# atomicarchitects/equiformer

Measured on AMD Instinct MI355X. Metric: molecules/sec (train step) QM9 L_max=2, 6 blocks, higher is better.
Workload: dtype f32; 1 GPU; QM9 graph_attention_transformer_nonlinear_l2 train step (radius graph + fwd + L1 + bwd + AdamW), 128 molecules/GPU x 18 atoms, r=5.0, num_basis=128, alpha_drop=0.2; global_batch=128, nodes_per_gpu=2304, edges_per_gpu=25354, parallelism=dp1, matrix_mode=split, hip_graph=True, hip_graph_replays=463, hip_graph_eager_steps=3

## Files before the change

equiformer_amd/csrc/gemmx.hip:

```cpp
#include <climits>
#include "sfcx_common.h"

namespace {

constexpr int GX_BK = 32;
constexpr int GX_LDK = 40;
constexpr int GX_T = 64;
constexpr int GX_ROW = GX_T * GX_LDK;
constexpr int GX_MAXP = 24;

typedef __bf16 bf16x4_t __attribute__((ext_vector_type(4)));

struct GRows {
  const float* base;
  int d, ld, inner;
};

struct GXP {
  GRows A, B, C;
  const float* bias;
  float* cs;
  float* Cw;
  int ldc;
  int M, N, K;
  int accumulate, kind;
  int vecA, vecB;
  int steps_per_split;
};
static_assert(sizeof(GXP) * GX_MAXP + 4 * (2 * GX_MAXP + 3) <= 4000, "kernarg segment");
struct GXGroup {
  int n;
  int woff[GX_MAXP + 1];
  GXP p[GX_MAXP];
};

__device__ __forceinline__ int flat_problem(const GXGroup& g, int b) {
  int pi = 0;
#pragma unroll
  for (int j = 1; j < GX_MAXP; ++j) pi += (int)((unsigned)(g.woff[j] - 1 - b) >> 31);
  return pi;
}

template <int NP>
__device__ __forceinline__ void split_n(const float* v, int n, __bf16 (*p)[8]) {
#pragma unroll
  for (int j = 0; j < 8; ++j) {
    if (j >= n) break;
    float r = v[j];
#pragma unroll
    for (int q = 0; q < NP; ++q) {
      const __bf16 h = (__bf16)r;
      p[q][j] = h;
      if (q + 1 < NP) r = r - (float)h;
    }
  }
}

template <int NP>
struct LoaderKC {
  float4 v[2];
  long roff[2];
  bool rv[2];
  __device__ __forceinline__ void init(const GRows& R, int x0, int X) {
    const int xr0 = threadIdx.x >> 3;
#pragma unroll
    for (int pass = 0; pass < 2; ++pass) {
      const int x = x0 + xr0 + 32 * pass;
      rv[pass] = x < X;
      roff[pass] = row_off2(rv[pass] ? x : x0, R.d, R.ld, R.inner);
    }
  }
  int krem;
  template <bool VEC>
  __device__ __forceinline__ void issue(const GRows& R, int k0, int K) {
    const int k = k0 + 4 * (threadIdx.x & 7);
    krem = K - k;
    if constexpr (VEC) {
      const int kc = krem > 0 ? k : 0;
#pragma unroll
      for (int pass = 0; pass < 2; ++pass) v[pass] = *reinterpret_cast<const float4*>(R.base + roff[pass] + kc);
    } else {
#pragma unroll
      for (int pass = 0; pass < 2; ++pass) {
        const float* const p = R.base + roff[pass];
        v[pass] = make_float4(p[min(k, K - 1)], p[min(k + 1, K - 1)], p[min(k + 2, K - 1)], p[min(k + 3, K - 1)]);
      }
    }
  }
  __device__ __forceinline__ void commit(__bf16* __restrict__ T) const {
    const int kq = threadIdx.x & 7, xr0 = threadIdx.x >> 3;
#pragma unroll
    for (int pass = 0; pass < 2; ++pass) {
      float f[4] = {v[pass].x, v[pass].y, v[pass].z, v[pass].w};
#pragma unroll
      for (int e = 0; e < 4; ++e)
        if (!(rv[pass] && e < krem)) f[e] = 0.f;
      __bf16 p[NP][8];
      split_n<NP>(f, 4, p);
#pragma unroll
      for (int q = 0; q < NP; ++q)
        *reinterpret_cast<bf16x4_t*>(T + q * GX_ROW + (xr0 + 32 * pass) * GX_LDK + 4 * kq) =
            bf16x4_t{p[q][0], p[q][1], p[q][2], p[q][3]};
    }
  }
};

template <int NP>
struct LoaderKS {
  float v[8];
  float cs, cc;
  int kleft;
  int kb, q, rem;
  __device__ __forceinline__ void init(const GRows& R, int k_first) {
    cs = 0.f, cc = 0.f;
    kb = k_first + 8 * (threadIdx.x >> 6);
    q = kb / R.d;
    rem = kb - q * R.d;
  }
  __device__ __forceinline__ void issue(const GRows& R, int K, int x0, int X) {
    const int x = x0 + (threadIdx.x & 63);
    const bool xv = x < X;
    const int nv = K - kb;
    kleft = xv ? nv : -1;
    const float* const p = R.base + (xv ? x : x0) + (nv > 0 ? (long)q * R.ld + (long)rem * R.inner : 0L);
    const int wrap = R.ld - R.d * R.inner;
    int rel = 0, r = rem;
#pragma unroll
    for (int j = 0; j < 8; ++j) {
      v[j] = p[j < nv ? rel : 0];
      rel += R.inner;
      if (++r == R.d) r = 0, rel += wrap;
    }
    const int q32 = GX_BK / R.d, r32 = GX_BK - q32 * R.d;
    kb += GX_BK, q += q32, rem += r32;
    if (rem >= R.d) rem -= R.d, ++q;
  }
  __device__ __forceinline__ void commit(__bf16* __restrict__ T, bool want_cs) {
    const int x = threadIdx.x & 63, kg = threadIdx.x >> 6;
#pragma unroll
    for (int j = 0; j < 8; ++j)
      if (j >= kleft) v[j] = 0.f;
    if (want_cs) {
#pragma unroll
      for (int j = 0; j < 8; ++j) {
        const float y = v[j] - cc, t = cs + y;
        cc = (t - cs) - y, cs = t;
      }
    }
    __bf16 p[NP][8];
    split_n<NP>(v, 8, p);
#pragma unroll
    for (int q_ = 0; q_ < NP; ++q_)
      *reinterpret_cast<bf16x8*>(T + q_ * GX_ROW + x * GX_LDK + 8 * kg) =
          bf16x8{p[q_][0], p[q_][1], p[q_][2], p[q_][3], p[q_][4], p[q_][5], p[q_][6], p[q_][7]};
  }
};

template <int NA, int NB>
__device__ __forceinline__ void gx_mma(const __bf16* __restrict__ As, const __bf16* __restrict__ Bs, int wm0, int wn0,
                                       f32x16& acc) {
  const int lane = threadIdx.x & 63, r = lane & 31, hi = lane >> 5;
#pragma unroll
  for (int kt = 0; kt < GX_BK / 16; ++kt) {
    bf16x8 a[NA], b[NB];
#pragma unroll
    for (int q = 0; q < NA; ++q) a[q] = *reinterpret_cast<const bf16x8*>(As + q * GX_ROW + (wm0 + r) * GX_LDK + 16 * kt + 8 * hi);
#pragma unroll
    for (int q = 0; q < NB; ++q) b[q] = *reinterpret_cast<const bf16x8*>(Bs + q * GX_ROW + (wn0 + r) * GX_LDK + 16 * kt + 8 * hi);
    mma_terms<NA, NB>(a, b, acc);
  }
}

constexpr int GX_ST_LD = 36;
constexpr int GX_ST_FLOATS = 16 * GX_ST_LD;
template <typename RowPtr>
__device__ __forceinline__ void gx_store_tile16(const f32x16& acc, float* __restrict__ T, const int row0, const int M, const int col0,
                                                const int N, const bool accumulate, const int lane, RowPtr rowptr) {
  const int r = lane & 31, hi = lane >> 5, c4 = 4 * (lane & 7), rr = lane >> 3;
#pragma unroll
  for (int half = 0; half < 2; ++half) {
    __builtin_amdgcn_fence(__ATOMIC_ACQ_REL, "wavefront");
    __builtin_amdgcn_wave_barrier();
#pragma unroll
    for (int q8 = 0; q8 < 8; ++q8) T[((q8 & 3) + 8 * (q8 >> 2) + 4 * hi) * GX_ST_LD + r] = acc[8 * half + q8];
    __builtin_amdgcn_fence(__ATOMIC_ACQ_REL, "wavefront");
    __builtin_amdgcn_wave_barrier();
#pragma unroll
    for (int k = 0; k < 2; ++k) {
      const int lr = rr + 8 * k, grow = row0 + 16 * half + lr;
      f32x4 v = *reinterpret_cast<const f32x4*>(T + lr * GX_ST_LD + c4);
      if (grow < M && col0 + c4 < N) {
        float* const p = rowptr(grow) + (col0 + c4);
        if (accumulate) {
          const f32x4 o = *reinterpret_cast<const f32x4*>(p);
          v[0] += o[0], v[1] += o[1], v[2] += o[2], v[3] += o[3];
        }
        *reinterpret_cast<f32x4*>(p) = v;
      }
    }
  }
}

template <int MODE, int BKIND, bool VEC>
__global__ __launch_bounds__(256) void gemmx_rows_kernel(const GXGroup g_byval) {
  KERNARG_IN_PLACE(GXGroup);
  constexpr int NA = Planes<MODE>::A, NB = Planes<MODE>::W;
  const int pi = flat_problem(g, (int)blockIdx.x);
  const GXP& P = g.p[pi];
  const int local = (int)blockIdx.x - g.woff[pi], tiles_n = (P.N + GX_T - 1) / GX_T;
  const int mt = local / tiles_n;
  const int m0 = mt * GX_T, n0 = (local - mt * tiles_n) * GX_T;
  __shared__ __attribute__((aligned(16))) __bf16 As[2][NA * GX_ROW];
  __shared__ __attribute__((aligned(16))) __bf16 Bs[2][NB * GX_ROW];
  const int wave = threadIdx.x >> 6;
  const int wm0 = (wave >> 1) * 32, wn0 = (wave & 1) * 32;
  f32x16 acc;
#pragma unroll
  for (int q = 0; q < 16; ++q) acc[q] = 0.f;

  LoaderKC<NA> la;
  LoaderKC<NB> lbk;
  LoaderKS<NB> lbs;
  la.init(P.A, m0, P.M);
  la.template issue<VEC>(P.A, 0, P.K);
  if constexpr (BKIND == 1) {
    lbk.init(P.B, n0, P.N);
    lbk.template issue<VEC>(P.B, 0, P.K);
  } else {
    lbs.init(P.B, 0);
    lbs.issue(P.B, P.K, n0, P.N);
  }
  la.commit(As[0]);
  if constexpr (BKIND == 1) lbk.commit(Bs[0]);
  else lbs.commit(Bs[0], false);
  __syncthreads();
  int cur = 0;
  for (int k0 = 0; k0 < P.K; k0 += GX_BK) {
    const bool more = k0 + GX_BK < P.K;
    if (more) {
      la.template issue<VEC>(P.A, k0 + GX_BK, P.K);
      if constexpr (BKIND == 1) lbk.template issue<VEC>(P.B, k0 + GX_BK, P.K);
      else lbs.issue(P.B, P.K, n0, P.N);
    }
    gx_mma<NA, NB>(As[cur], Bs[cur], wm0, wn0, acc);
    if (more) {
      la.commit(As[cur ^ 1]);
      if constexpr (BKIND == 1) lbk.commit(Bs[cur ^ 1]);
      else lbs.commit(Bs[cur ^ 1], false);
    }
    __syncthreads();
    cur ^= 1;
  }

  const int lane = threadIdx.x & 63, r = lane & 31, hi = lane >> 5;
  const int col = n0 + wn0 + r;
  const float bv = (P.bias && col < P.N) ? P.bias[col] : 0.f;
  const bool flat_c = P.C.d == 1;
  const SmallDiv cdiv(P.C.d);
  float* const cbase = const_cast<float*>(P.C.base);
  const int rb = m0 + wm0 + 4 * hi;
  static_assert(sizeof(As) >= 4 * GX_ST_FLOATS * sizeof(float), "the operand stages double as the store tiles");
  if (((P.C.ld | P.C.inner | P.N) & 3) == 0 && (reinterpret_cast<size_t>(cbase) & 15) == 0) {
#pragma unroll
    for (int q = 0; q < 16; ++q) acc[q] += bv;
    gx_store_tile16(acc, reinterpret_cast<float*>(&As[0][0]) + wave * GX_ST_FLOATS, m0 + wm0, P.M, n0 + wn0, P.N, P.accumulate != 0,
                    lane, [&](const int grow) {
                      if (flat_c) return cbase + (long)grow * P.C.ld;
                      const int qd = grow / P.C.d;
                      return cbase + (long)qd * P.C.ld + (long)(grow - qd * P.C.d) * P.C.inner;
                    });
    return;
  }
  if (col >= P.N) return;
  long off0;
  int rem0 = 0;
  if (flat_c) {
    off0 = (long)rb * P.C.ld;
  } else {
    const int qb = rb / P.C.d;
    rem0 = rb - qb * P.C.d;
    off0 = (long)qb * P.C.ld;
  }
#pragma unroll
  for (int q = 0; q < 16; ++q) {
    const int dr = (q & 3) + 8 * (q >> 2);
    if (rb + dr < P.M) {
      long off;
      if (flat_c) {
        off = off0 + (long)dr * P.C.ld;
      } else {
        const int t = rem0 + dr, dq = cdiv.div(t);
        off = off0 + (long)dq * P.C.ld + (long)(t - dq * P.C.d) * P.C.inner;
      }
      float* p = cbase + off + col;
      float v = acc[q] + bv;
      if (P.accumulate) v += *p;
      *p = v;
    }
  }
}

constexpr int GW_K = 64;
constexpr int GW_LDK = GW_K + 8;
constexpr int GW_ROW = GX_T * GW_LDK;

template <int NP>
struct LoaderWide {
  float4 v[GW_K / 16];
  int kv;
  __device__ __forceinline__ void issue(const GRows& R, int x0, int X, int K, bool two_level) {
    const int row = x0 + (threadIdx.x >> 2), q = threadIdx.x & 3;
    const bool rv = row < X;
    kv = rv ? K : 0;
    const long off = two_level ? row_off2(rv ? row : x0, R.d, R.ld, R.inner) : (long)(rv ? row : x0) * R.ld;
#pragma unroll
    for (int j = 0; j < GW_K / 16; ++j) {
      const int k = 4 * (q + 4 * j);
      v[j] = *reinterpret_cast<const float4*>(R.base + off + (k < K ? k : 0));
    }
  }
  __device__ __forceinline__ void commit(__bf16* __restrict__ T) const {
    const int row = threadIdx.x >> 2, q = threadIdx.x & 3;
#pragma unroll
    for (int j = 0; j < GW_K / 16; ++j) {
      const bool ok = 4 * (q + 4 * j) < kv;
      const float f[4] = {ok ? v[j].x : 0.f, ok ? v[j].y : 0.f, ok ? v[j].z : 0.f, ok ? v[j].w : 0.f};
      __bf16 p[NP][8];
      split_n<NP>(f, 4, p);
#pragma unroll
      for (int pl = 0; pl < NP; ++pl)
        *reinterpret_cast<bf16x4_t*>(T + pl * GW_ROW + row * GW_LDK + 4 * (q + 4 * j)) = bf16x4_t{p[pl][0], p[pl][1], p[pl][2], p[pl][3]};
    }
  }
};

template <int MODE>
__global__ __launch_bounds__(256) void gemmx_rows_wide_kernel(const GXGroup g_byval) {
  KERNARG_IN_PLACE(GXGroup);
  constexpr int NA = Planes<MODE>::A, NB = Planes<MODE>::W;
  const GXP& P = g.p[blockIdx.z];
  const int m0 = blockIdx.x * GX_T;
  if (m0 >= P.M) return;
  __shared__ __attribute__((aligned(16))) __bf16 As[NA * GW_ROW];
  __shared__ __attribute__((aligned(16))) __bf16 Bs[NB * GW_ROW];
  __shared__ __attribute__((aligned(16))) float St[4 * GX_ST_FLOATS];
  const int wave = threadIdx.x >> 6, lane = threadIdx.x & 63, r = lane & 31, hi = lane >> 5;
  const int wm0 = (wave >> 1) * 32, wn0 = (wave & 1) * 32;
  LoaderWide<NA> la;
  LoaderWide<NB> lb;
  la.issue(P.A, m0, P.M, P.K, true);
  lb.issue(P.B, 0, P.N, P.K, false);
  la.commit(As);
  const bool flat_c = P.C.d == 1;
  const SmallDiv cdiv(P.C.d);
  float* const cbase = const_cast<float*>(P.C.base);
  const int rb = m0 + wm0 + 4 * hi;
  long off0;
  int rem0 = 0;
  if (flat_c) {
    off0 = (long)rb * P.C.ld;
  } else {
    const int qb = rb / P.C.d;
    rem0 = rb - qb * P.C.d;
    off0 = (long)qb * P.C.ld;
  }
  const int nkt = (P.K + 15) / 16;
  const bool vec_c = ((P.C.ld | P.C.inner | P.N) & 3) == 0 && (reinterpret_cast<size_t>(cbase) & 15) == 0;
  for (int n0 = 0; n0 < P.N; n0 += GX_T) {
    __syncthreads();
    lb.commit(Bs);
    __syncthreads();
    if (n0 + GX_T < P.N) lb.issue(P.B, n0 + GX_T, P.N, P.K, false);
    f32x16 acc;
#pragma unroll
    for (int q = 0; q < 16; ++q) acc[q] = 0.f;
#pragma unroll
    for (int kt = 0; kt < GW_K / 16; ++kt) {
      if (kt < nkt) {
        bf16x8 a[NA], b[NB];
#pragma unroll
        for (int q = 0; q < NA; ++q) a[q] = *reinterpret_cast<const bf16x8*>(As + q * GW_ROW + (wm0 + r) * GW_LDK + 16 * kt + 8 * hi);
#pragma unroll
        for (int q = 0; q < NB; ++q) b[q] = *reinterpret_cast<const bf16x8*>(Bs + q * GW_ROW + (wn0 + r) * GW_LDK + 16 * kt + 8 * hi);
        mma_terms<NA, NB>(a, b, acc);
      }
    }
    const int col = n0 + wn0 + r;
    if (vec_c) {
      const float bv = (P.bias && col < P.N) ? P.bias[col] : 0.f;
#pragma unroll
      for (int q = 0; q < 16; ++q) acc[q] += bv;
      gx_store_tile16(acc, St + wave * GX_ST_FLOATS, m0 + wm0, P.M, n0 + wn0, P.N, P.accumulate != 0, lane, [&](const int grow) {
        if (flat_c) return cbase + (long)grow * P.C.ld;
        const int qd = grow / P.C.d;
        return cbase + (long)qd * P.C.ld + (long)(grow - qd * P.C.d) * P.C.inner;
      });
    } else if (col < P.N) {
      const float bv = P.bias ? P.bias[col] : 0.f;
#pragma unroll
      for (int q = 0; q < 16; ++q) {
        const int dr = (q & 3) + 8 * (q >> 2);
        if (rb + dr < P.M) {
          long off;
          if (flat_c) {
            off = off0 + (long)dr * P.C.ld;
          } else {
            const int t = rem0 + dr, dq = cdiv.div(t);
            off = off0 + (long)dq * P.C.ld + (long)(t - dq * P.C.d) * P.C.inner;
          }
          float* p = cbase + off + col;
          float v = acc[q] + bv;
          if (P.accumulate) v += *p;
          *p = v;
        }
      }
    }
  }
}

template <int MODE>
__global__ __launch_bounds__(256) void gemmx_tn_kernel(const GXGroup g_byval) {
  KERNARG_IN_PLACE(GXGroup);
  constexpr int NA = Planes<MODE>::A;
  const int pi = flat_problem(g, (int)blockIdx.x);
  const GXP& P = g.p[pi];
  const int local = (int)blockIdx.x - g.woff[pi], tiles_n = (P.N + GX_T - 1) / GX_T;
  const int tiles = ((P.M + GX_T - 1) / GX_T) * tiles_n;
  const int bz = local / tiles, tile = local - bz * tiles;
  const int mt = tile / tiles_n, nt = tile - mt * tiles_n;
  const int m0 = mt * GX_T, n0 = nt * GX_T;
  __shared__ __attribute__((aligned(16))) __bf16 As[2][NA * GX_ROW];
  __shared__ __attribute__((aligned(16))) __bf16 Bs[2][NA * GX_ROW];
  const int wave = threadIdx.x >> 6;
  const int wm0 = (wave >> 1) * 32, wn0 = (wave & 1) * 32;
  f32x16 acc;
#pragma unroll
  for (int q = 0; q < 16; ++q) acc[q] = 0.f;
  const int total = (P.K + GX_BK - 1) / GX_BK;
  const int s_beg = bz * P.steps_per_split;
  const int s_end = min(total, s_beg + P.steps_per_split);
  if (s_beg >= s_end) return;
  const bool csA = P.kind == 3 && P.cs != nullptr && nt == 0;
  const bool csB = P.kind == 2 && P.cs != nullptr && mt == 0;
  LoaderKS<NA> la, lb;
  la.init(P.A, s_beg * GX_BK);
  lb.init(P.B, s_beg * GX_BK);
  la.issue(P.A, P.K, m0, P.M);
  lb.issue(P.B, P.K, n0, P.N);
  la.commit(As[0], csA);
  lb.commit(Bs[0], csB);
  __syncthreads();
  int cur = 0;
  for (int s = s_beg; s < s_end; ++s) {
    const bool more = s + 1 < s_end;
    if (more) {
      la.issue(P.A, P.K, m0, P.M);
      lb.issue(P.B, P.K, n0, P.N);
    }
    gx_mma<NA, NA>(As[cur], Bs[cur], wm0, wn0, acc);
    if (more) {
      la.commit(As[cur ^ 1], csA);
      lb.commit(Bs[cur ^ 1], csB);
    }
    __syncthreads();
    cur ^= 1;
  }
  {
    const int x = threadIdx.x & 63;
    if (csA && m0 + x < P.M) atomicAdd(P.cs + m0 + x, la.cs);
    if (csB && n0 + x < P.N) atomicAdd(P.cs + n0 + x, lb.cs);
  }
  const int lane = threadIdx.x & 63, r = lane & 31, hi = lane >> 5;
  const int col = n0 + wn0 + r;
  if (col >= P.N) return;
#pragma unroll
  for (int q = 0; q < 16; ++q) {
    const int row = m0 + wm0 + (q & 3) + 8 * (q >> 2) + 4 * hi;
    if (row < P.M) atomicAdd(P.Cw + (long)row * P.ldc + col, acc[q]);
  }
}

inline bool aligned16(const void* p) { return (reinterpret_cast<uintptr_t>(p) & 15) == 0; }
inline bool rows_vec_ok(const float* base, const eqf_rows& r) { return aligned16(base) && (r.ld % 4 == 0) && (r.inner % 4 == 0); }

static int g_gemmx_tn_minsteps = 8;

}

extern "C" {

int eqf_gemmx_group(const eqf_gemm_desc* d, int n, int mode, void* stream) {
  if (!d || n < 1 || n > GX_MAXP || mode < 0 || mode > 2) return EQF_E_BADARG;
  hipStream_t st = (hipStream_t)stream;
  for (int i = 0; i < n; ++i) {
    if (d[i].kind < 0 || d[i].kind > 3) return EQF_E_BADARG;
    if (!d[i].A || !d[i].B || !d[i].C || d[i].ra.d < 1 || d[i].rc.d < 1) return EQF_E_BADARG;
    if (d[i].kind < 2 && d[i].K < 1) return EQF_E_BADARG;
  }
  static thread_local GXGroup G;
  for (int kind = 0; kind < 2; ++kind) {
    memset(&G, 0, sizeof G);
    int maxm = 0, big = 0, wide_ok = 1, vec_ok = 1, wg = 0;
    double flops = 0, bytes = 0;
    for (int i = 0; i < n; ++i) {
      if (d[i].kind != kind || d[i].M <= 0 || d[i].N <= 0) continue;
      GXP& P = G.p[G.n];
      G.woff[G.n++] = wg;
      wg += eqf_cdiv(d[i].M, GX_T) * eqf_cdiv(d[i].N, GX_T);
      P.A = {d[i].A, d[i].ra.d, d[i].ra.ld, d[i].ra.inner};
      P.B = {d[i].B, 1, d[i].ldb, 0};
      P.C = {d[i].C, d[i].rc.d, d[i].rc.ld, d[i].rc.inner};
      P.bias = d[i].bias;
      P.M = d[i].M, P.N = d[i].N, P.K = d[i].K, P.accumulate = d[i].accumulate, P.kind = kind;
      P.vecA = rows_vec_ok(d[i].A, d[i].ra);
      P.vecB = aligned16(d[i].B) && d[i].ldb % 4 == 0;
      if (P.K % 4 != 0 || !P.vecA || (kind == 1 && !P.vecB)) vec_ok = 0;
      if (!(kind == 1 && P.K <= GW_K && P.K % 4 == 0 && P.vecA && P.vecB && P.M >= 8192 && P.N >= 2 * GX_T)) wide_ok = 0;
      if (eqf_cdiv(P.M, GX_T) > maxm) maxm = eqf_cdiv(P.M, GX_T);
      if (P.M >= 32768 / 2 + 1) big = 1;
      flops += 2.0 * P.M * (double)P.N * P.K;
      bytes += 4.0 * ((double)P.M * P.K + (double)P.K * P.N + (double)P.M * P.N);
    }
    if (G.n == 0) continue;
    const bool wide = kind == 1 && wide_ok;
    for (int i = G.n; i <= GX_MAXP; ++i) G.woff[i] = i == G.n ? wg : INT_MAX;
    const dim3 grid = wide ? dim3(maxm, 1, G.n) : dim3(wg, 1, 1);
    const int pid = eqf_prof_begin(kind == 0 ? (big ? "gemmx_group_kn_edge" : "gemmx_group_kn_node")
                                             : (big ? "gemmx_group_nk_edge" : "gemmx_group_nk_node"), st, flops, bytes);
#define GX_ROWS(M_)                                                                                              \
  do {                                                                                                           \
    if (wide) {                                                                                                  \
      hipLaunchKernelGGL((gemmx_rows_wide_kernel<M_>), grid, dim3(256), 0, st, G);                              \
    } else if (kind == 0) {                                                                                      \
      if (vec_ok) hipLaunchKernelGGL((gemmx_rows_kernel<M_, 0, true>), grid, dim3(256), 0, st, G);              \
      else hipLaunchKernelGGL((gemmx_rows_kernel<M_, 0, false>), grid, dim3(256), 0, st, G);                    \
    } else {                                                                                                     \
      if (vec_ok) hipLaunchKernelGGL((gemmx_rows_kernel<M_, 1, true>), grid, dim3(256), 0, st, G);              \
      else hipLaunchKernelGGL((gemmx_rows_kernel<M_, 1, false>), grid, dim3(256), 0, st, G);                    \
    }                                                                                                            \
  } while (0)
    if (mode == 0) GX_ROWS(0);
    else if (mode == 1) GX_ROWS(1);
    else GX_ROWS(2);
#undef GX_ROWS
    eqf_prof_end(pid, st);
    EQF_CHECK_LAUNCH();
  }
  {
    memset(&G, 0, sizeof G);
    int big = 0, wg = 0;
    double flops = 0, bytes = 0;
    for (int i = 0; i < n; ++i) {
      if (d[i].kind != 2 && d[i].kind != 3) continue;
      if (d[i].M <= 0 || d[i].N <= 0 || d[i].K <= 0) continue;
      GXP& P = G.p[G.n];
      P.A = {d[i].A, d[i].ra.d, d[i].ra.ld, d[i].ra.inner};
      P.B = {d[i].B, d[i].rc.d, d[i].rc.ld, d[i].rc.inner};
      P.Cw = d[i].C, P.ldc = d[i].ldb, P.M = d[i].M, P.N = d[i].N, P.K = d[i].K, P.kind = d[i].kind;
      P.cs = const_cast<float*>(d[i].bias);
      const int tiles = eqf_cdiv(P.M, GX_T) * eqf_cdiv(P.N, GX_T);
      const int total_steps = eqf_cdiv(P.K, GX_BK);
      int ksplit = 1024 / (tiles > 0 ? tiles : 1);
      const int max_split = eqf_cdiv(total_steps, g_gemmx_tn_minsteps);
      if (ksplit > max_split) ksplit = max_split;
      if (ksplit < 1) ksplit = 1;
      P.steps_per_split = eqf_cdiv(total_steps, ksplit);
      ksplit = eqf_cdiv(total_steps, P.steps_per_split);
      G.woff[G.n] = wg;
      wg += tiles * ksplit;
      G.n++;
      if (P.K >= 32768 / 2 + 1) big = 1;
      flops += 2.0 * P.M * (double)P.N * P.K;
      bytes += 4.0 * ((double)P.K * P.M + (double)P.K * P.N + (double)P.M * P.N);
    }
    if (G.n > 0) {
      for (int i = G.n; i <= GX_MAXP; ++i) G.woff[i] = i == G.n ? wg : INT_MAX;
      const dim3 grid(wg, 1, 1);
      const int pid = eqf_prof_begin(big ? "gemmx_group_tn_edge" : "gemmx_group_tn_node", st, flops, bytes);
      if (mode == 0) hipLaunchKernelGGL((gemmx_tn_kernel<0>), grid, dim3(256), 0, st, G);
      else if (mode == 1) hipLaunchKernelGGL((gemmx_tn_kernel<1>), grid, dim3(256), 0, st, G);
      else hipLaunchKernelGGL((gemmx_tn_kernel<2>), grid, dim3(256), 0, st, G);
      eqf_prof_end(pid, st);
      EQF_CHECK_LAUNCH();
    }
  }
  return 0;
}

}
```

equiformer_amd/lib.py:

```python
import ctypes
import os

_HERE = os.path.dirname(os.path.abspath(__file__))
LIB_PATH = os.path.join(_HERE, "libequiformer_hip.so")
if os.environ.get("EQF_LIB_VARIANT"):
    LIB_PATH = os.path.join(_HERE, "libequiformer_hip_%s.so" % os.environ["EQF_LIB_VARIANT"])

EQF_MAX_SEG = 8
EQF_MAX_PATHS = 72
EQF_L3_ODD = 0x100

c_fp = ctypes.c_void_p
c_int = ctypes.c_int


class EqfIrreps(ctypes.Structure):
    _fields_ = [("nseg", c_int), ("l", c_int * EQF_MAX_SEG), ("mul", c_int * EQF_MAX_SEG), ("odd", c_int * EQF_MAX_SEG)]


class EqfRows(ctypes.Structure):
    _fields_ = [("d", c_int), ("ld", c_int), ("inner", c_int)]


class EqfGemmDesc(ctypes.Structure):
# ... 86 lines not shown
                                       c_int, c_fp],
    "eqf_sfcx_pack": [_PP, c_fp, _P_PATHS, _P_IRR, c_int, c_int, c_fp, c_fp],
    "eqf_sfcx_fwd": [c_fp, c_fp, c_fp, _P_PATHS, c_fp, c_fp, c_fp, c_fp, _P_IRR, c_fp, c_int, c_int, c_int, c_fp],
    "eqf_sfcx_bwd_data": [c_fp, c_fp, c_fp, _P_PATHS, c_fp, c_fp, _P_IRR, c_fp, c_int, c_fp, c_fp, c_fp, c_int, c_int, c_fp],
    "eqf_sfcx_bwd_weight": [c_fp, c_fp, c_fp, _P_PATHS, c_fp, _P_IRR, c_fp, c_int, _PP, c_fp, c_int, c_int, c_fp],
    "eqf_layernorm_fwd": [c_fp, c_fp, c_fp, c_fp, c_fp, c_fp, c_int, _P_IRR, _f, c_fp],
    "eqf_layernorm_bwd": [c_fp, c_fp, c_fp, c_fp, c_fp, c_fp, c_fp, c_fp, c_int, _P_IRR, c_fp],
    "eqf_layernorm_wgrad_group": [ctypes.POINTER(EqfLnWgradDesc), c_int, c_fp],
    "eqf_add_layernorm_fwd": [c_fp, c_fp, c_fp, c_fp, c_fp, c_fp, c_fp, c_fp, c_int, _P_IRR, _f, c_fp],
    "eqf_add_layernorm_bwd": [c_fp, c_fp, c_fp, c_fp, c_fp, c_fp, c_fp, c_fp, c_fp, c_int, _P_IRR, c_fp],
    "eqf_graphnorm_fwd": [c_fp, c_fp, c_fp, c_fp, c_fp, c_fp, c_fp, c_fp, c_fp, c_fp, c_fp, c_int, c_int, _P_IRR, _f, c_fp],
    "eqf_graphnorm_bwd": [c_fp, c_fp, c_fp, c_fp, c_fp, c_fp, c_fp, c_fp, c_fp, c_fp, c_fp, c_fp, c_fp, c_fp, c_int, c_int,
                          _P_IRR, c_fp],
    "eqf_gate_fwd": [c_fp, c_fp, c_int, c_int, _P_IRR, _f, _f, c_fp],
    "eqf_gate_bwd": [c_fp, c_fp, c_fp, c_int, c_int, _P_IRR, _f, _f, c_fp],
    "eqf_silu_fwd": [c_fp, c_fp, _long, _f, c_fp],
    "eqf_silu_bwd": [c_fp, c_fp, c_fp, _long, _f, c_fp],
    "eqf_lnsilu_fwd": [c_fp, c_fp, c_fp, c_fp, c_int, c_int, _f, c_fp],
    "eqf_lnsilu_group_fwd": [c_fp, c_fp, c_fp, c_fp, c_int, c_int, c_int, _f, c_fp],
    "eqf_lnsilu_group_bwd": [c_fp, c_fp, c_fp, c_fp, c_fp, c_fp, c_fp, c_int, c_int, c_int, _f, c_fp],
    "eqf_fold_weight_fwd": [c_fp, c_fp, c_fp, c_fp, c_fp, c_int, c_fp],
    "eqf_fold_weight_bwd": [c_fp, c_fp, c_fp, c_fp, c_fp, c_fp, c_fp, c_int, c_fp],
    "eqf_embed_fwd": [c_fp, c_fp, c_fp, c_fp, c_int, c_int, c_int, c_fp],
    "eqf_embed_bwd": [c_fp, c_fp, c_fp, c_fp, c_int, c_int, c_int, c_fp],
    "eqf_gather_add_fwd": [c_fp, c_fp, c_fp, c_fp, c_fp, c_int, c_int, c_fp],
    "eqf_segment_sum": [c_fp, c_fp, c_fp, c_fp, c_int, c_int, _f, c_int, c_fp],
    "eqf_segment_sum_pair": [c_fp, c_fp, c_fp, c_fp, c_fp, c_fp, c_fp, c_int, c_int, c_fp],
    "eqf_segment_bcast": [c_fp, c_fp, c_fp, c_int, c_int, _f, c_fp],
    "eqf_kv_split": [c_fp, c_fp, c_fp, c_int, c_int, c_fp, c_fp],
    "eqf_kv_merge": [c_fp, c_fp, c_fp, c_int, c_int, c_fp, c_fp],
    "eqf_dp_logits_fwd": [c_fp, c_fp, c_fp, c_fp, c_int, c_int, c_fp, c_fp],
    "eqf_dp_logits_bwd": [c_fp, c_fp, c_fp, c_fp, c_fp, c_fp, c_int, c_int, c_fp, c_fp],
    "eqf_vec_sh": [c_fp, c_fp, c_int, c_int, _f, c_fp, c_fp],
    "eqf_edgedeg_fold_fwd": [c_fp, c_fp, c_fp, c_fp, c_fp, _P_EDEG, c_fp, c_fp, c_fp],
    "eqf_edgedeg_fold_bwd": [c_fp, c_fp, c_fp, c_fp, c_fp, _P_EDEG, c_fp, c_fp, c_fp, c_fp, c_fp, c_fp, c_fp],
    "eqf_edgedeg_scatter_fwd": [c_fp, c_fp, c_fp, c_fp, _P_EDEG, _f, c_fp, c_int, c_int, c_fp],
    "eqf_edgedeg_scatter_bwd": [c_fp, c_fp, c_fp, c_fp, _P_EDEG, _f, c_fp, c_fp, c_int, c_int, c_fp],
    "eqf_segment_scale": [c_fp, c_fp, c_fp, c_fp, c_int, c_int, c_fp],
    "eqf_segment_droppath": [c_fp, c_fp, c_fp, c_int, c_int, _f, _f, _u64, c_fp, _u64, c_fp],
    "eqf_irreps_dropout": [c_fp, c_fp, c_int, _P_IRR, c_int, _f, _f, _u64, c_fp, _u64, c_fp],
    "eqf_dtp_fwd": [c_fp, c_fp, c_fp, _P_PATHS, c_fp, c_int, c_fp],
    "eqf_dtp_bwd": [c_fp, c_fp, c_fp, _P_PATHS, c_fp, c_fp, c_fp, c_fp, c_int, c_fp],
    "eqf_alpha_fwd": [c_fp, c_fp, c_fp, c_int, c_int, c_int, _f, c_fp],
    "eqf_alpha_bwd": [c_fp, c_fp, c_fp, c_fp, c_fp, c_int, c_int, c_int, _f, c_fp],
    "eqf_attn_aggregate_fwd": [c_fp, c_fp, c_fp, c_fp, c_fp, c_int, c_int, _P_IRR, _f, _u64, c_fp],
    "eqf_attn_aggregate_bwd": [c_fp, c_fp, c_fp, c_fp, c_fp, c_fp, c_int, c_int, _P_IRR, _f, _u64, c_fp],
    "eqf_attn_aggregate_fwd_dseed": [c_fp, c_fp, c_fp, c_fp, c_fp, c_int, c_int, _P_IRR, _f, _u64, c_fp, c_fp],
    "eqf_attn_aggregate_bwd_dseed": [c_fp, c_fp, c_fp, c_fp, c_fp, c_fp, c_int, c_int, _P_IRR, _f, _u64, c_fp, c_fp],
    "eqf_silu_bwd2": [c_fp, c_fp, c_fp, c_fp, c_fp, _long, _f, c_fp],
    "eqf_gate_bwd2": [c_fp, c_fp, c_fp, c_fp, c_fp, c_int, c_int, _P_IRR, _f, _f, c_fp],
    "eqf_lnsilu_group_bwd2": [c_fp, c_fp, c_fp, c_fp, c_fp, c_fp, c_fp, c_fp, c_fp, c_int, c_int, c_int, _f, c_fp],
    "eqf_layernorm_bwd2": [c_fp, c_fp, c_fp, c_fp, c_fp, c_fp, c_fp, c_int, _P_IRR, _f, c_fp],
    "eqf_alpha_bwd2": [c_fp, c_fp, c_fp, c_fp, c_fp, c_fp, c_fp, c_int, c_int, c_int, _f, c_fp],
    "eqf_attn_aggregate_bwd2": [c_fp, c_fp, c_fp, c_fp, c_fp, c_fp, c_fp, c_fp, c_fp, c_int, c_int, _P_IRR, _f, _u64,
                                c_fp],
    "eqf_rbf_expnorm_bwd2": [c_fp, c_fp, c_fp, c_int, c_int, c_fp, c_fp, _f, _f, c_fp, c_fp, c_fp],
    "eqf_rbf_gaussian_bwd2": [c_fp, c_fp, c_fp, c_int, c_int, c_fp, c_fp, c_fp, c_fp, _f, c_fp, c_fp, c_fp, c_fp, c_fp,
                              c_fp, c_fp],
    "eqf_rbf_bessel_bwd2": [c_fp, c_fp, c_fp, c_int, c_int, c_fp, _f, c_fp, c_fp, c_fp, c_fp],
    "eqf_edge_geom_bwd2": [c_fp, c_fp, c_fp, c_fp, c_int, c_int, c_fp, c_fp, c_fp, c_fp],
    "eqf_dens_corrupt": [c_fp, c_fp, c_fp, c_int, _f, _f, _f, _u64, c_fp, c_fp, c_fp, c_fp, c_fp, c_fp],
    "eqf_dens_loss_fwd": [c_fp, c_fp, c_fp, c_fp, c_fp, c_fp, c_fp, c_fp, c_int, c_int, _d, _d, _d, c_fp, c_fp, c_fp],
    "eqf_dens_loss_bwd": [c_fp, c_fp, c_fp, c_fp, c_fp, c_fp, c_fp, c_fp, c_fp, c_fp, c_int, c_int, _d, _d, _d, c_fp, c_fp,
                          c_fp],
    "eqf_is2rs_perturb": [c_fp, c_fp, c_fp, c_int, c_fp, c_int, _f, _f, _f, _u64, c_fp, c_fp, c_fp, c_fp, c_fp],
    "eqf_is2rs_loss_fwd": [c_fp, c_fp, c_fp, c_fp, c_fp, c_fp, c_int, c_fp, c_fp, c_int, c_int, _d, _d, _d, _d, _d, _d, _d, _d,
                           _d, c_fp, c_fp, c_fp],
    "eqf_is2rs_loss_bwd": [c_fp, c_fp, c_fp, c_fp, c_fp, c_fp, c_fp, c_int, c_fp, c_fp, c_fp, c_int, c_int, _d, _d, _d, _d, _d,
                           _d, _d, _d, c_fp, c_fp, c_fp],
    "eqf_metrics_accumulate": [c_fp, c_fp, c_int, c_fp, c_fp, c_fp, c_int, _d, _d, _d, c_fp, c_fp],
    "eqf_prof_enable": [ctypes.c_char_p],
    "eqf_prof_report": [ctypes.c_char_p, c_int],
}

RESTYPES = {"eqf_sfcx_packed_numel": ctypes.c_long}

_lib = None


class HipLibraryError(RuntimeError):
    pass


def load():
    global _lib
    if _lib is not None:
        return _lib
    if not os.path.exists(LIB_PATH):
        raise HipLibraryError(
            "libequiformer_hip.so not found at %s -- build it with `python -m equiformer_amd.build` "
            "(there is no CPU fallback for the hot path)" % LIB_PATH)
    lib = ctypes.CDLL(LIB_PATH)
    lib.eqf_version.restype = ctypes.c_char_p
    lib.eqf_version.argtypes = []
    for name, argtypes in SIGNATURES.items():
        fn = getattr(lib, name)
        fn.restype = RESTYPES.get(name, c_int)
        fn.argtypes = argtypes
    _check_build(lib)
    _lib = lib
    return lib


def _check_build(lib):
    csrc = os.path.join(_HERE, "csrc")
    if not os.path.isdir(csrc):
        return
    ver = lib.eqf_version().decode()
    built = ver.split("src=")[-1] if "src=" in ver else "unknown"
    from . import build as _build
    want = _build.source_hash()
    if built != want:
        msg = ("libequiformer_hip.so was built from sources with hash %s, the sources beside it hash to %s -- rebuild with "
               "`python -m equiformer_amd.build`" % (built, want))
        if os.environ.get("EQF_ALLOW_STALE_LIB") == "1":
            import warnings
            warnings.warn(msg)
        else:
            raise HipLibraryError(msg)


def built_hash():
    ver = version()
    return ver.split("src=")[-1] if "src=" in ver else "unknown"


def version():
    return load().eqf_version().decode()


_fn_cache = {}


def call(name, *args):
    fn = _fn_cache.get(name)
    if fn is None:
        fn = _fn_cache[name] = getattr(load(), name)
    rc = fn(*args)
    if rc != 0:
        raise HipLibraryError("%s failed with code %d" % (name, rc))


def prof_enable(filter_substring):
    load().eqf_prof_enable(None if filter_substring is None else filter_substring.encode())


def prof_report():
    buf = ctypes.create_string_buffer(1 << 16)
    n = load().eqf_prof_report(buf, len(buf))
    out = {}
    if n > 0:
        for line in buf.value.decode().splitlines():
            name, cnt, ms, fl, by = line.split()
            out[name] = dict(launches=int(float(cnt)), total_ms=float(ms), flops=float(fl), bytes=float(by))
    return out


def make_irreps(segments, parities=None):
    segments = list(segments)
    if len(segments) > EQF_MAX_SEG:
        raise ValueError("too many irreps segments")
    s = EqfIrreps()
    s.nseg = len(segments)
    for i, (mul, l) in enumerate(segments):
        s.l[i], s.mul[i] = int(l), int(mul)
        s.odd[i] = 1 if parities is not None and parities[i] == -1 else 0
    return s
```

include/equiformer_hip_dev.h:

```cpp
#ifndef EQUIFORMER_HIP_DEV_H
#define EQUIFORMER_HIP_DEV_H

#include "equiformer_hip.h"

#ifdef __cplusplus
extern "C" {
#endif

int eqf_sfcx_dev_plan(int kind, const eqf_dtp_paths* paths, const eqf_irreps* out1_irreps, int n2, int E, int mode,
                      char* buf, int buflen);
int eqf_sfcx_dev_set(int key, int value);
int eqf_sfcx_dev_served(int family);

#ifdef __cplusplus
}
#endif
#endif
```

Measured before the change: 15460 molecules/s.

## Add two-deep register prefetch ring to gemmx kernels and N-split wide kernel

Moves loader staging registers into per-stage structs so the rows and TN GEMM kernels can keep two k-steps of global loads in flight (a ring of depth 2) when the K loop is long enough, hiding global load latency behind MMA. The wide kernel is changed to a flat grid that splits N into chunks chosen to reduce workgroup-slot tail waste, and its store staging buffer is halved so three workgroups fit per CU in split mode. A dev switch lets both features be turned off. The deeper prefetch raises register pressure, which may lower occupancy.

Measured after the change: 15610 molecules/s, median of 6. About the same (+0.9%).

```diff
diff --git a/equiformer_amd/csrc/gemmx.hip b/equiformer_amd/csrc/gemmx.hip
--- a/equiformer_amd/csrc/gemmx.hip
+++ b/equiformer_amd/csrc/gemmx.hip
@@ -56,9 +56,12 @@
   }
 }
 
+struct KCStage {
+  float4 v[2];
+  int krem;
+};
 template <int NP>
 struct LoaderKC {
-  float4 v[2];
   long roff[2];
   bool rv[2];
   __device__ __forceinline__ void init(const GRows& R, int x0, int X) {
@@ -70,31 +73,30 @@
       roff[pass] = row_off2(rv[pass] ? x : x0, R.d, R.ld, R.inner);
     }
   }
-  int krem;
   template <bool VEC>
-  __device__ __forceinline__ void issue(const GRows& R, int k0, int K) {
+  __device__ __forceinline__ void issue(KCStage& s, const GRows& R, int k0, int K) const {
     const int k = k0 + 4 * (threadIdx.x & 7);
-    krem = K - k;
+    s.krem = K - k;
     if constexpr (VEC) {
-      const int kc = krem > 0 ? k : 0;
-#pragma unroll
-      for (int pass = 0; pass < 2; ++pass) v[pass] = *reinterpret_cast<const float4*>(R.base + roff[pass] + kc);
+      const int kc = s.krem > 0 ? k : 0;
+#pragma unroll
+      for (int pass = 0; pass < 2; ++pass) s.v[pass] = *reinterpret_cast<const float4*>(R.base + roff[pass] + kc);
     } else {
 #pragma unroll
       for (int pass = 0; pass < 2; ++pass) {
         const float* const p = R.base + roff[pass];
-        v[pass] = make_float4(p[min(k, K - 1)], p[min(k + 1, K - 1)], p[min(k + 2, K - 1)], p[min(k + 3, K - 1)]);
-      }
-    }
-  }
-  __device__ __forceinline__ void commit(__bf16* __restrict__ T) const {
+        s.v[pass] = make_float4(p[min(k, K - 1)], p[min(k + 1, K - 1)], p[min(k + 2, K - 1)], p[min(k + 3, K - 1)]);
+      }
+    }
+  }
+  __device__ __forceinline__ void commit(const KCStage& s, __bf16* __restrict__ T) const {
     const int kq = threadIdx.x & 7, xr0 = threadIdx.x >> 3;
 #pragma unroll
     for (int pass = 0; pass < 2; ++pass) {
-      float f[4] = {v[pass].x, v[pass].y, v[pass].z, v[pass].w};
+      float f[4] = {s.v[pass].x, s.v[pass].y, s.v[pass].z, s.v[pass].w};
 #pragma unroll
       for (int e = 0; e < 4; ++e)
-        if (!(rv[pass] && e < krem)) f[e] = 0.f;
+        if (!(rv[pass] && e < s.krem)) f[e] = 0.f;
       __bf16 p[NP][8];
       split_n<NP>(f, 4, p);
 #pragma unroll
@@ -105,11 +107,13 @@
   }
 };
 
+struct KSStage {
+  float v[8];
+  int kleft;
+};
 template <int NP>
 struct LoaderKS {
-  float v[8];
   float cs, cc;
-  int kleft;
   int kb, q, rem;
   __device__ __forceinline__ void init(const GRows& R, int k_first) {
     cs = 0.f, cc = 0.f;
@@ -117,17 +121,17 @@
     q = kb / R.d;
     rem = kb - q * R.d;
   }
-  __device__ __forceinline__ void issue(const GRows& R, int K, int x0, int X) {
+  __device__ __forceinline__ void issue(KSStage& s, const GRows& R, int K, int x0, int X) {
     const int x = x0 + (threadIdx.x & 63);
     const bool xv = x < X;
     const int nv = K - kb;
-    kleft = xv ? nv : -1;
+    s.kleft = xv ? nv : -1;
     const float* const p = R.base + (xv ? x : x0) + (nv > 0 ? (long)q * R.ld + (long)rem * R.inner : 0L);
     const int wrap = R.ld - R.d * R.inner;
     int rel = 0, r = rem;
 #pragma unroll
     for (int j = 0; j < 8; ++j) {
-      v[j] = p[j < nv ? rel : 0];
+      s.v[j] = p[j < nv ? rel : 0];
       rel += R.inner;
       if (++r == R.d) r = 0, rel += wrap;
     }
@@ -135,11 +139,11 @@
     kb += GX_BK, q += q32, rem += r32;
     if (rem >= R.d) rem -= R.d, ++q;
   }
-  __device__ __forceinline__ void commit(__bf16* __restrict__ T, bool want_cs) {
+  __device__ __forceinline__ void commit(const KSStage& s, __bf16* __restrict__ T, bool want_cs) {
     const int x = threadIdx.x & 63, kg = threadIdx.x >> 6;
-#pragma unroll
-    for (int j = 0; j < 8; ++j)
-      if (j >= kleft) v[j] = 0.f;
+    float v[8];
+#pragma unroll
+    for (int j = 0; j < 8; ++j) v[j] = j >= s.kleft ? 0.f : s.v[j];
     if (want_cs) {
 #pragma unroll
       for (int j = 0; j < 8; ++j) {
@@ -173,21 +177,23 @@
 
 constexpr int GX_ST_LD = 36;
 constexpr int GX_ST_FLOATS = 16 * GX_ST_LD;
-template <typename RowPtr>
+template <int ROWS = 16, typename RowPtr>
 __device__ __forceinline__ void gx_store_tile16(const f32x16& acc, float* __restrict__ T, const int row0, const int M, const int col0,
                                                 const int N, const bool accumulate, const int lane, RowPtr rowptr) {
+  static_assert(ROWS == 16 || ROWS == 8, "accumulator registers come in groups of 4 rows + 4 hi, 8 apart");
+  constexpr int NQ = ROWS / 2;
   const int r = lane & 31, hi = lane >> 5, c4 = 4 * (lane & 7), rr = lane >> 3;
 #pragma unroll
-  for (int half = 0; half < 2; ++half) {
+  for (int half = 0; half < 32 / ROWS; ++half) {
     __builtin_amdgcn_fence(__ATOMIC_ACQ_REL, "wavefront");
     __builtin_amdgcn_wave_barrier();
 #pragma unroll
-    for (int q8 = 0; q8 < 8; ++q8) T[((q8 & 3) + 8 * (q8 >> 2) + 4 * hi) * GX_ST_LD + r] = acc[8 * half + q8];
+    for (int q8 = 0; q8 < NQ; ++q8) T[((q8 & 3) + 8 * (q8 >> 2) + 4 * hi) * GX_ST_LD + r] = acc[NQ * half + q8];
     __builtin_amdgcn_fence(__ATOMIC_ACQ_REL, "wavefront");
     __builtin_amdgcn_wave_barrier();
 #pragma unroll
-    for (int k = 0; k < 2; ++k) {
-      const int lr = rr + 8 * k, grow = row0 + 16 * half + lr;
+    for (int k = 0; k < ROWS / 8; ++k) {
+      const int lr = rr + 8 * k, grow = row0 + ROWS * half + lr;
       f32x4 v = *reinterpret_cast<const f32x4*>(T + lr * GX_ST_LD + c4);
       if (grow < M && col0 + c4 < N) {
         float* const p = rowptr(grow) + (col0 + c4);
@@ -201,7 +207,7 @@
   }
 }
 
-template <int MODE, int BKIND, bool VEC>
+template <int MODE, int BKIND, bool VEC, int DEPTH>
 __global__ __launch_bounds__(256) void gemmx_rows_kernel(const GXGroup g_byval) {
   KERNARG_IN_PLACE(GXGroup);
   constexpr int NA = Planes<MODE>::A, NB = Planes<MODE>::W;
@@ -221,35 +227,57 @@
   LoaderKC<NA> la;
   LoaderKC<NB> lbk;
   LoaderKS<NB> lbs;
+  KCStage sa[DEPTH], sbk[DEPTH];
+  KSStage sbs[DEPTH];
   la.init(P.A, m0, P.M);
-  la.template issue<VEC>(P.A, 0, P.K);
-  if constexpr (BKIND == 1) {
-    lbk.init(P.B, n0, P.N);
-    lbk.template issue<VEC>(P.B, 0, P.K);
-  } else {
-    lbs.init(P.B, 0);
-    lbs.issue(P.B, P.K, n0, P.N);
-  }
-  la.commit(As[0]);
-  if constexpr (BKIND == 1) lbk.commit(Bs[0]);
-  else lbs.commit(Bs[0], false);
+  if constexpr (BKIND == 1) lbk.init(P.B, n0, P.N);
+  else lbs.init(P.B, 0);
+  auto issue = [&](const int j, const int k0) {
+    la.template issue<VEC>(sa[j], P.A, k0, P.K);
+    if constexpr (BKIND == 1) lbk.template issue<VEC>(sbk[j], P.B, k0, P.K);
+    else lbs.issue(sbs[j], P.B, P.K, n0, P.N);
+  };
+  auto commit = [&](const int j, const int buf) {
+    la.commit(sa[j], As[buf]);
+    if constexpr (BKIND == 1) lbk.commit(sbk[j], Bs[buf]);
+    else lbs.commit(sbs[j], Bs[buf], false);
+  };
+#pragma unroll
+  for (int j = 0; j < DEPTH; ++j) issue(j, j * GX_BK);
+  commit(0, 0);
   __syncthreads();
   int cur = 0;
-  for (int k0 = 0; k0 < P.K; k0 += GX_BK) {
-    const bool more = k0 + GX_BK < P.K;
-    if (more) {
-      la.template issue<VEC>(P.A, k0 + GX_BK, P.K);
-      if constexpr (BKIND == 1) lbk.template issue<VEC>(P.B, k0 + GX_BK, P.K);
-      else lbs.issue(P.B, P.K, n0, P.N);
-    }
-    gx_mma<NA, NB>(As[cur], Bs[cur], wm0, wn0, acc);
-    if (more) {
-      la.commit(As[cur ^ 1]);
-      if constexpr (BKIND == 1) lbk.commit(Bs[cur ^ 1]);
-      else lbs.commit(Bs[cur ^ 1], false);
-    }
-    __syncthreads();
-    cur ^= 1;
+  if constexpr (DEPTH == 1) {
+    for (int k0 = 0; k0 < P.K; k0 += GX_BK) {
+      const bool more = k0 + GX_BK < P.K;
+      if (more) issue(0, k0 + GX_BK);
+      gx_mma<NA, NB>(As[cur], Bs[cur], wm0, wn0, acc);
+      if (more) commit(0, cur ^ 1);
+      __syncthreads();
+      cur ^= 1;
+    }
+  } else {
+    const int nsteps = (P.K + GX_BK - 1) / GX_BK;
+    int s = 0;
+    for (; s + DEPTH < nsteps; s += DEPTH) {
+#pragma unroll
+      for (int j = 0; j < DEPTH; ++j) {
+        issue(j, (s + j + DEPTH) * GX_BK);
+        gx_mma<NA, NB>(As[cur], Bs[cur], wm0, wn0, acc);
+        commit((j + 1) % DEPTH, cur ^ 1);
+        __syncthreads();
+        cur ^= 1;
+      }
+    }
+#pragma unroll
+    for (int j = 0; j < DEPTH; ++j) {
+      if (s + j < nsteps) {
+        gx_mma<NA, NB>(As[cur], Bs[cur], wm0, wn0, acc);
+        if (s + j + 1 < nsteps) commit((j + 1) % DEPTH, cur ^ 1);
+        __syncthreads();
+        cur ^= 1;
+      }
+    }
   }
 
   const int lane = threadIdx.x & 63, r = lane & 31, hi = lane >> 5;
@@ -303,6 +331,9 @@
 constexpr int GW_K = 64;
 constexpr int GW_LDK = GW_K + 8;
 constexpr int GW_ROW = GX_T * GW_LDK;
+constexpr int GW_ST_FLOATS = 8 * GX_ST_LD;
+constexpr int GW_MAXCHUNKS = 3;
+constexpr int GW_SLOTS = 3 * 256;
 
 template <int NP>
 struct LoaderWide {
@@ -338,18 +369,23 @@
 __global__ __launch_bounds__(256) void gemmx_rows_wide_kernel(const GXGroup g_byval) {
   KERNARG_IN_PLACE(GXGroup);
   constexpr int NA = Planes<MODE>::A, NB = Planes<MODE>::W;
-  const GXP& P = g.p[blockIdx.z];
-  const int m0 = blockIdx.x * GX_T;
-  if (m0 >= P.M) return;
+  const int pi = flat_problem(g, (int)blockIdx.x);
+  const GXP& P = g.p[pi];
+  const int local = (int)blockIdx.x - g.woff[pi];
+  const int chunks = ((P.N + GX_T - 1) / GX_T + P.steps_per_split - 1) / P.steps_per_split;
+  const int mt = local / chunks;
+  const int m0 = mt * GX_T, n_beg = (local - mt * chunks) * P.steps_per_split * GX_T;
+  const int n_end = min(P.N, n_beg + P.steps_per_split * GX_T);
   __shared__ __attribute__((aligned(16))) __bf16 As[NA * GW_ROW];
   __shared__ __attribute__((aligned(16))) __bf16 Bs[NB * GW_ROW];
-  __shared__ __attribute__((aligned(16))) float St[4 * GX_ST_FLOATS];
+  __shared__ __attribute__((aligned(16))) float St[4 * GW_ST_FLOATS];
+  static_assert(MODE != 0 || sizeof(As) + sizeof(Bs) + sizeof(St) <= 160 * 1024 / 3, "split mode: three workgroups per CU");
   const int wave = threadIdx.x >> 6, lane = threadIdx.x & 63, r = lane & 31, hi = lane >> 5;
   const int wm0 = (wave >> 1) * 32, wn0 = (wave & 1) * 32;
   LoaderWide<NA> la;
   LoaderWide<NB> lb;
   la.issue(P.A, m0, P.M, P.K, true);
-  lb.issue(P.B, 0, P.N, P.K, false);
+  lb.issue(P.B, n_beg, P.N, P.K, false);
   la.commit(As);
   const bool flat_c = P.C.d == 1;
   const SmallDiv cdiv(P.C.d);
@@ -366,11 +402,11 @@
   }
   const int nkt = (P.K + 15) / 16;
   const bool vec_c = ((P.C.ld | P.C.inner | P.N) & 3) == 0 && (reinterpret_cast<size_t>(cbase) & 15) == 0;
-  for (int n0 = 0; n0 < P.N; n0 += GX_T) {
+  for (int n0 = n_beg; n0 < n_end; n0 += GX_T) {
     __syncthreads();
     lb.commit(Bs);
     __syncthreads();
-    if (n0 + GX_T < P.N) lb.issue(P.B, n0 + GX_T, P.N, P.K, false);
+    if (n0 + GX_T < n_end) lb.issue(P.B, n0 + GX_T, P.N, P.K, false);
     f32x16 acc;
 #pragma unroll
     for (int q = 0; q < 16; ++q) acc[q] = 0.f;
@@ -390,7 +426,7 @@
       const float bv = (P.bias && col < P.N) ? P.bias[col] : 0.f;
 #pragma unroll
       for (int q = 0; q < 16; ++q) acc[q] += bv;
-      gx_store_tile16(acc, St + wave * GX_ST_FLOATS, m0 + wm0, P.M, n0 + wn0, P.N, P.accumulate != 0, lane, [&](const int grow) {
+      gx_store_tile16<8>(acc, St + wave * GW_ST_FLOATS, m0 + wm0, P.M, n0 + wn0, P.N, P.accumulate != 0, lane, [&](const int grow) {
         if (flat_c) return cbase + (long)grow * P.C.ld;
         const int qd = grow / P.C.d;
         return cbase + (long)qd * P.C.ld + (long)(grow - qd * P.C.d) * P.C.inner;
@@ -418,7 +454,7 @@
   }
 }
 
-template <int MODE>
+template <int MODE, int DEPTH>
 __global__ __launch_bounds__(256) void gemmx_tn_kernel(const GXGroup g_byval) {
   KERNARG_IN_PLACE(GXGroup);
   constexpr int NA = Planes<MODE>::A;
@@ -443,27 +479,53 @@
   const bool csA = P.kind == 3 && P.cs != nullptr && nt == 0;
   const bool csB = P.kind == 2 && P.cs != nullptr && mt == 0;
   LoaderKS<NA> la, lb;
+  KSStage sa[DEPTH], sb[DEPTH];
   la.init(P.A, s_beg * GX_BK);
   lb.init(P.B, s_beg * GX_BK);
-  la.issue(P.A, P.K, m0, P.M);
-  lb.issue(P.B, P.K, n0, P.N);
-  la.commit(As[0], csA);
-  lb.commit(Bs[0], csB);
+  const int k_end = DEPTH == 1 ? P.K : min(P.K, s_end * GX_BK);
+  auto issue = [&](const int j) {
+    la.issue(sa[j], P.A, k_end, m0, P.M);
+    lb.issue(sb[j], P.B, k_end, n0, P.N);
+  };
+  auto commit = [&](const int j, const int buf) {
+    la.commit(sa[j], As[buf], csA);
+    lb.commit(sb[j], Bs[buf], csB);
+  };
+#pragma unroll
+  for (int j = 0; j < DEPTH; ++j) issue(j);
+  commit(0, 0);
   __syncthreads();
   int cur = 0;
-  for (int s = s_beg; s < s_end; ++s) {
-    const bool more = s + 1 < s_end;
-    if (more) {
-      la.issue(P.A, P.K, m0, P.M);
-      lb.issue(P.B, P.K, n0, P.N);
-    }
-    gx_mma<NA, NA>(As[cur], Bs[cur], wm0, wn0, acc);
-    if (more) {
-      la.commit(As[cur ^ 1], csA);
-      lb.commit(Bs[cur ^ 1], csB);
-    }
-    __syncthreads();
-    cur ^= 1;
+  if constexpr (DEPTH == 1) {
+    for (int s = s_beg; s < s_end; ++s) {
+      const bool more = s + 1 < s_end;
+      if (more) issue(0);
+      gx_mma<NA, NA>(As[cur], Bs[cur], wm0, wn0, acc);
+      if (more) commit(0, cur ^ 1);
+      __syncthreads();
+      cur ^= 1;
+    }
+  } else {
+    int s = s_beg;
+    for (; s + DEPTH < s_end; s += DEPTH) {
+#pragma unroll
+      for (int j = 0; j < DEPTH; ++j) {
+        issue(j);
+        gx_mma<NA, NA>(As[cur], Bs[cur], wm0, wn0, acc);
+        commit((j + 1) % DEPTH, cur ^ 1);
+        __syncthreads();
+        cur ^= 1;
+      }
+    }
+#pragma unroll
+    for (int j = 0; j < DEPTH; ++j) {
+      if (s + j < s_end) {
+        gx_mma<NA, NA>(As[cur], Bs[cur], wm0, wn0, acc);
+        if (s + j + 1 < s_end) commit((j + 1) % DEPTH, cur ^ 1);
+        __syncthreads();
+        cur ^= 1;
+      }
+    }
   }
   {
     const int x = threadIdx.x & 63;
@@ -485,9 +547,19 @@
 
 static int g_gemmx_tn_minsteps = 8;
 
+constexpr int GX_RING = 2;
+constexpr int GX_RING_MINSTEPS = 5;
+static int g_gemmx_dev_plain = 0;
+
 }
 
 extern "C" {
+
+int eqf_gemmx_dev_set(int key, int value) {
+  if (key != 1 || (value != 0 && value != 1)) return EQF_E_BADARG;
+  g_gemmx_dev_plain = value;
+  return 0;
+}
 
 int eqf_gemmx_group(const eqf_gemm_desc* d, int n, int mode, void* stream) {
   if (!d || n < 1 || n > GX_MAXP || mode < 0 || mode > 2) return EQF_E_BADARG;
@@ -500,7 +572,7 @@
   static thread_local GXGroup G;
   for (int kind = 0; kind < 2; ++kind) {
     memset(&G, 0, sizeof G);
-    int maxm = 0, big = 0, wide_ok = 1, vec_ok = 1, wg = 0;
+    int maxsteps = 0, big = 0, wide_ok = 1, vec_ok = 1, wg = 0;
     double flops = 0, bytes = 0;
     for (int i = 0; i < n; ++i) {
       if (d[i].kind != kind || d[i].M <= 0 || d[i].N <= 0) continue;
@@ -516,39 +588,66 @@
       P.vecB = aligned16(d[i].B) && d[i].ldb % 4 == 0;
       if (P.K % 4 != 0 || !P.vecA || (kind == 1 && !P.vecB)) vec_ok = 0;
       if (!(kind == 1 && P.K <= GW_K && P.K % 4 == 0 && P.vecA && P.vecB && P.M >= 8192 && P.N >= 2 * GX_T)) wide_ok = 0;
-      if (eqf_cdiv(P.M, GX_T) > maxm) maxm = eqf_cdiv(P.M, GX_T);
+      if (eqf_cdiv(P.K, GX_BK) > maxsteps) maxsteps = eqf_cdiv(P.K, GX_BK);
       if (P.M >= 32768 / 2 + 1) big = 1;
       flops += 2.0 * P.M * (double)P.N * P.K;
       bytes += 4.0 * ((double)P.M * P.K + (double)P.K * P.N + (double)P.M * P.N);
     }
     if (G.n == 0) continue;
     const bool wide = kind == 1 && wide_ok;
+    if (wide) {
+      int best = 1;
+      double best_waste = 0;
+      for (int c = 1; c <= (g_gemmx_dev_plain ? 1 : GW_MAXCHUNKS); ++c) {
+        wg = 0;
+        for (int i = 0; i < G.n; ++i) {
+          const int tn = eqf_cdiv(G.p[i].N, GX_T);
+          wg += eqf_cdiv(G.p[i].M, GX_T) * eqf_cdiv(tn, eqf_cdiv(tn, c));
+        }
+        const double waste = (double)eqf_cdiv(wg, GW_SLOTS) * GW_SLOTS / wg;
+        if (c == 1 || waste < best_waste) best = c, best_waste = waste;
+      }
+      wg = 0;
+      for (int i = 0; i < G.n; ++i) {
+        const int tn = eqf_cdiv(G.p[i].N, GX_T);
+        G.p[i].steps_per_split = eqf_cdiv(tn, best);
+        G.woff[i] = wg;
+        wg += eqf_cdiv(G.p[i].M, GX_T) * eqf_cdiv(tn, G.p[i].steps_per_split);
+      }
+    }
     for (int i = G.n; i <= GX_MAXP; ++i) G.woff[i] = i == G.n ? wg : INT_MAX;
-    const dim3 grid = wide ? dim3(maxm, 1, G.n) : dim3(wg, 1, 1);
+    const dim3 grid(wg, 1, 1);
+    const bool ring = !g_gemmx_dev_plain && maxsteps >= GX_RING_MINSTEPS;
     const int pid = eqf_prof_begin(kind == 0 ? (big ? "gemmx_group_kn_edge" : "gemmx_group_kn_node")
                                              : (big ? "gemmx_group_nk_edge" : "gemmx_group_nk_node"), st, flops, bytes);
+#define GX_ROWS_D(M_, B_, V_)                                                                                    \
+  do {                                                                                                           \
+    if (ring) hipLaunchKernelGGL((gemmx_rows_kernel<M_, B_, V_, GX_RING>), grid, dim3(256), 0, st, G);          \
+    else hipLaunchKernelGGL((gemmx_rows_kernel<M_, B_, V_, 1>), grid, dim3(256), 0, st, G);                     \
+  } while (0)
 #define GX_ROWS(M_)                                                                                              \
   do {                                                                                                           \
     if (wide) {                                                                                                  \
       hipLaunchKernelGGL((gemmx_rows_wide_kernel<M_>), grid, dim3(256), 0, st, G);                              \
     } else if (kind == 0) {                                                                                      \
-      if (vec_ok) hipLaunchKernelGGL((gemmx_rows_kernel<M_, 0, true>), grid, dim3(256), 0, st, G);              \
-      else hipLaunchKernelGGL((gemmx_rows_kernel<M_, 0, false>), grid, dim3(256), 0, st, G);                    \
+      if (vec_ok) GX_ROWS_D(M_, 0, true);                                                                        \
+      else GX_ROWS_D(M_, 0, false);                                                                              \
     } else {                                                                                                     \
-      if (vec_ok) hipLaunchKernelGGL((gemmx_rows_kernel<M_, 1, true>), grid, dim3(256), 0, st, G);              \
-      else hipLaunchKernelGGL((gemmx_rows_kernel<M_, 1, false>), grid, dim3(256), 0, st, G);                    \
+      if (vec_ok) GX_ROWS_D(M_, 1, true);                                                                        \
+      else GX_ROWS_D(M_, 1, false);                                                                              \
     }                                                                                                            \
   } while (0)
     if (mode == 0) GX_ROWS(0);
     else if (mode == 1) GX_ROWS(1);
     else GX_ROWS(2);
 #undef GX_ROWS
+#undef GX_ROWS_D
     eqf_prof_end(pid, st);
     EQF_CHECK_LAUNCH();
   }
   {
     memset(&G, 0, sizeof G);
-    int big = 0, wg = 0;
+    int big = 0, wg = 0, maxsteps = 0;
     double flops = 0, bytes = 0;
     for (int i = 0; i < n; ++i) {
       if (d[i].kind != 2 && d[i].kind != 3) continue;
@@ -566,6 +665,7 @@
       if (ksplit < 1) ksplit = 1;
       P.steps_per_split = eqf_cdiv(total_steps, ksplit);
       ksplit = eqf_cdiv(total_steps, P.steps_per_split);
+      if (P.steps_per_split > maxsteps) maxsteps = P.steps_per_split;
       G.woff[G.n] = wg;
       wg += tiles * ksplit;
       G.n++;
@@ -577,9 +677,16 @@
       for (int i = G.n; i <= GX_MAXP; ++i) G.woff[i] = i == G.n ? wg : INT_MAX;
       const dim3 grid(wg, 1, 1);
       const int pid = eqf_prof_begin(big ? "gemmx_group_tn_edge" : "gemmx_group_tn_node", st, flops, bytes);
-      if (mode == 0) hipLaunchKernelGGL((gemmx_tn_kernel<0>), grid, dim3(256), 0, st, G);
-      else if (mode == 1) hipLaunchKernelGGL((gemmx_tn_kernel<1>), grid, dim3(256), 0, st, G);
-      else hipLaunchKernelGGL((gemmx_tn_kernel<2>), grid, dim3(256), 0, st, G);
+      const bool ring = !g_gemmx_dev_plain && maxsteps >= GX_RING_MINSTEPS;
+#define GX_TN(M_)                                                                                        \
+  do {                                                                                                   \
+    if (ring) hipLaunchKernelGGL((gemmx_tn_kernel<M_, GX_RING>), grid, dim3(256), 0, st, G);            \
+    else hipLaunchKernelGGL((gemmx_tn_kernel<M_, 1>), grid, dim3(256), 0, st, G);                       \
+  } while (0)
+      if (mode == 0) GX_TN(0);
+      else if (mode == 1) GX_TN(1);
+      else GX_TN(2);
+#undef GX_TN
       eqf_prof_end(pid, st);
       EQF_CHECK_LAUNCH();
     }
diff --git a/equiformer_amd/lib.py b/equiformer_amd/lib.py
--- a/equiformer_amd/lib.py
+++ b/equiformer_amd/lib.py
@@ -192,6 +192,11 @@
     pass
 
 
+DEV_SIGNATURES = {
+    "eqf_gemmx_dev_set": [c_int, c_int],
+}
+
+
 def load():
     global _lib
     if _lib is not None:
@@ -206,6 +211,10 @@
     for name, argtypes in SIGNATURES.items():
         fn = getattr(lib, name)
         fn.restype = RESTYPES.get(name, c_int)
+        fn.argtypes = argtypes
+    for name, argtypes in DEV_SIGNATURES.items():
+        fn = getattr(lib, name)
+        fn.restype = c_int
         fn.argtypes = argtypes
     _check_build(lib)
     _lib = lib
diff --git a/include/equiformer_hip_dev.h b/include/equiformer_hip_dev.h
--- a/include/equiformer_hip_dev.h
+++ b/include/equiformer_hip_dev.h
@@ -10,6 +10,7 @@
 int eqf_sfcx_dev_plan(int kind, const eqf_dtp_paths* paths, const eqf_irreps* out1_irreps, int n2, int E, int mode,
                       char* buf, int buflen);
 int eqf_sfcx_dev_set(int key, int value);
+int eqf_gemmx_dev_set(int key, int value);
 int eqf_sfcx_dev_served(int family);
 
 #ifdef __cplusplus
```
